# evenrose/CMDIAD

Measured on AMD Instinct MI355X. Metric: images/sec end-to-end (extract+distill+kNN score), higher is better.
Workload: dtype bf16; 1 GPU; configs[1]: DINO ViT-B/8 + Point-MAE predict (DoubleRGBPointFeatures: both modalities are extracted, this method has no distillation step at test time; the `mtfi_step` leg times the method that has one), 224x224 RGB + 24576-point clouds (1024 groups x 128), batch 32/GPU, bagel-sized banks (xyz 76518x768, rgb 19129x768); batch_per_gpu=32, rotating_input_batches=4, bank=single, hip_graphs=True, search_operands=bf16 (fp32 accumulate, exact fp32 re-score of the winner), weights=seeded random init (no checkpoints offline)

## Files before the change

cmdiad_amd/csrc/mlp_fused.hip:

```cpp
#include "gemm_core.h"
#include "launch.h"

namespace {

using namespace gemm;

constexpr int kC = 384, kHid = 1536, kBM = 128, kWaves = 8;
constexpr int kChunks = kHid / 64;
constexpr int kKT1 = kC / BK;
constexpr int kPer = kKT1 + kC / 64;
constexpr int kSlots = 6, kAhead = kSlots - 1;
static_assert(kPer % kSlots == 0, "the slot of a piece depends on its place in the chunk only");
constexpr int kPieceBytes = 64 * BK * 2;
constexpr int kXbWave = kKT1 * 16 * BK * 2;
constexpr int kHOff = kWaves * kXbWave;
constexpr int kRingOff = kHOff + kWaves * 2048;
constexpr int kLdsBytes = kRingOff + kSlots * kPieceBytes;
static_assert(kLdsBytes == 160 * 1024, "LDS budget");

struct MlpParams {
    int M;
    const bf16_t* xb;
    const float* row_scale;
    const bf16_t* w1;
    const float* b1;
    const bf16_t* w2;
    const float* b2;
    float* x;
    bf16_t* ln_xb;
    float* ln_part;
    const float* add2;
};

__device__ __forceinline__ void mlp_barrier() { asm volatile("s_barrier" ::: "memory"); }

__device__ __forceinline__ float half_row_sum8(float v)
{
    v += __builtin_bit_cast(float, __builtin_amdgcn_update_dpp(0, __builtin_bit_cast(int, v), 0xB1, 0xF, 0xF, false));
    v += __builtin_bit_cast(float, __builtin_amdgcn_update_dpp(0, __builtin_bit_cast(int, v), 0x4E, 0xF, 0xF, false));
    v += __builtin_bit_cast(float, __builtin_amdgcn_update_dpp(0, __builtin_bit_cast(int, v), 0x141, 0xF, 0xF, false));
    return v;
}

template <bool LN_OUT>
__global__ __launch_bounds__(512, 1) void pmae_mlp_fused_kernel(MlpParams p)
{
    extern __shared__ __attribute__((aligned(16))) char lds[];
    const int lane = threadIdx.x & 63, wave = __builtin_amdgcn_readfirstlane(threadIdx.x >> 6);
    const int g = lane >> 4, r16 = lane & 15;
    const int mw = (int)blockIdx.x * kBM + wave * 16;
    char* xs = lds + wave * kXbWave;
    char* hs = lds + kHOff + wave * 2048;
    char* ring = lds + kRingOff;

    float rsc;
    f32x4 b1v[4];
    auto load_b1 = [&](int c) {
        const float* bp = p.b1 + c * 64 + g * 4;
#pragma unroll
        for (int j = 0; j < 4; ++j) asm volatile("global_load_dwordx4 %0, %1, off" : "=v"(b1v[j]) : "v"(bp + j * 16) : "memory");
    };
    {
        const float* rp = p.row_scale + min(mw + r16, p.M - 1);
        asm volatile("global_load_dword %0, %1, off" : "=v"(rsc) : "v"(rp) : "memory");
    }
    load_b1(0);
    const int sw_chunk = (lane & 7) ^ (lane >> 3);
#pragma unroll
    for (int e = 0; e < 2; ++e) {
        const bf16_t* src = p.xb + (size_t)min(mw + e * 8 + (lane >> 3), p.M - 1) * kC + sw_chunk * 8;
#pragma unroll
        for (int s = 0; s < kKT1; ++s)
            __builtin_amdgcn_global_load_lds((const __attribute__((address_space(1))) void*)(src + s * BK),
                                             (__attribute__((address_space(3))) void*)(xs + s * 2048 + e * 1024), 16, 0, 0);
    }
    const char* w1l = reinterpret_cast<const char*>(p.w1 + (size_t)(wave * 8 + (lane >> 3)) * kC + sw_chunk * 8);
    const char* w2l = reinterpret_cast<const char*>(p.w2 + (size_t)(wave * 8 + (lane >> 3)) * kHid + sw_chunk * 8);
    auto issue = [&](int c, int q) {
        const char* src = q < kKT1 ? w1l + ((size_t)c * 64 * kC + q * BK) * 2 : w2l + ((size_t)(q - kKT1) * 64 * kHid + c * BK) * 2;
        __builtin_amdgcn_global_load_lds((const __attribute__((address_space(1))) void*)src,
                                         (__attribute__((address_space(3))) void*)(ring + (q % kSlots) * kPieceBytes + wave * 1024), 16, 0, 0);
    };
#pragma unroll
    for (int q = 0; q < kAhead; ++q) issue(0, q);
    asm volatile("s_waitcnt vmcnt(4)" ::: "memory");
    mlp_barrier();

    auto ldf = [&](const char* tile, int row, int kk) { return *reinterpret_cast<const bf16x8*>(tile + lds_off(row, kk * 4 + g)); };
    auto step = [&](const char* wt, const bf16x8& a0, const bf16x8& a1, f32x4 (&acc)[4]) {
        bf16x8 wf[2][4];
#pragma unroll
        for (int kk = 0; kk < 2; ++kk)
#pragma unroll
            for (int j = 0; j < 4; ++j) wf[kk][j] = ldf(wt, j * 16 + r16, kk);
        __builtin_amdgcn_s_setprio(1);
#pragma unroll
        for (int kk = 0; kk < 2; ++kk)
#pragma unroll
            for (int j = 0; j < 4; ++j) acc[j] = mfma16(wf[kk][j], kk ? a1 : a0, acc[j]);
        __builtin_amdgcn_s_setprio(0);
    };

    f32x4 acc2[kC / 64][4];
#pragma unroll
    for (int nb = 0; nb < kC / 64; ++nb)
#pragma unroll
        for (int j = 0; j < 4; ++j) acc2[nb][j] = f32x4{0.f, 0.f, 0.f, 0.f};

    for (int c = 0; c < kChunks; ++c) {
        f32x4 acc1[4];
#pragma unroll
        for (int j = 0; j < 4; ++j) acc1[j] = f32x4{0.f, 0.f, 0.f, 0.f};
        bf16x8 h0, h1;
#pragma unroll
        for (int q = 0; q < kPer; ++q) {
            const int qn = q + kAhead < kPer ? q + kAhead : q + kAhead - kPer;
            const int cn = q + kAhead < kPer ? c : c + 1;
            const bool more = cn < kChunks;
            if (q == 7 && more) load_b1(c + 1);
            if (more) issue(cn, qn);
            const char* wt = ring + (q % kSlots) * kPieceBytes;
            if (q < kKT1) step(wt, ldf(xs + q * 2048, r16, 0), ldf(xs + q * 2048, r16, 1), acc1);
            else step(wt, h0, h1, acc2[q - kKT1]);
            if (!more) asm volatile("s_waitcnt vmcnt(0)" ::: "memory");
            else if (q >= 7 && q <= 10) asm volatile("s_waitcnt vmcnt(8)" ::: "memory");
            else asm volatile("s_waitcnt vmcnt(4)" ::: "memory");
            mlp_barrier();
            if (q == kKT1 - 1) {
                __builtin_amdgcn_sched_barrier(0);
#pragma unroll
                for (int j = 0; j < 4; ++j) {
                    f32x4 v = __builtin_elementwise_fma(acc1[j], f32x4{rsc, rsc, rsc, rsc}, b1v[j]);
                    v = gelu_erf4(v);
                    const bf16x4 hv = {f2bf(v[0]), f2bf(v[1]), f2bf(v[2]), f2bf(v[3])};
                    *reinterpret_cast<bf16x4*>(hs + lds_off(r16, 2 * j + (g >> 1)) + (g & 1) * 8) = hv;
                }
                h0 = ldf(hs, r16, 0);
                h1 = ldf(hs, r16, 1);
            }
        }
    }

    RowStore32 rs;
    rs.init(hs, lane);
    const bool full = mw + 16 <= p.M;
    const int m0r = mw + rs.R;
    const int ma = min(m0r, p.M - 1), mb = min(m0r + 8, p.M - 1);
#pragma unroll
    for (int nb = 0; nb < kC / 64; ++nb) {
        const int n0 = nb * 64;
        f32x4 bj[4];
#pragma unroll
        for (int j = 0; j < 4; ++j) bj[j] = *reinterpret_cast<const f32x4*>(p.b2 + n0 + j * 16 + g * 4);
        f32x4 o0[2], o1[2];
#pragma unroll
        for (int ch = 0; ch < 2; ++ch) {
            const int col = n0 + ch * 32 + rs.u * 4;
            const f32x4 r0 = *reinterpret_cast<const f32x4*>(p.x + (size_t)ma * kC + col);
            const f32x4 r1 = *reinterpret_cast<const f32x4*>(p.x + (size_t)mb * kC + col);
            f32x4 a0 = {0.f, 0.f, 0.f, 0.f}, a1 = a0;
            if (LN_OUT && p.add2) {
                a0 = *reinterpret_cast<const f32x4*>(p.add2 + (size_t)ma * kC + col);
                a1 = *reinterpret_cast<const f32x4*>(p.add2 + (size_t)mb * kC + col);
            }
            rs.park(acc2[nb][2 * ch] + bj[2 * ch], acc2[nb][2 * ch + 1] + bj[2 * ch + 1]);
            f32x4 t0, t1;
            rs.fetch(t0, t1);
            o0[ch] = t0 + r0;
            o1[ch] = t1 + r1;
            if (LN_OUT && p.add2) { o0[ch] += a0; o1[ch] += a1; }
            if (full || m0r < p.M) *reinterpret_cast<f32x4*>(p.x + (size_t)m0r * kC + col) = o0[ch];
            if (full || m0r + 8 < p.M) *reinterpret_cast<f32x4*>(p.x + (size_t)(m0r + 8) * kC + col) = o1[ch];
            if constexpr (LN_OUT) {
                const bf16x4 v0 = {f2bf(o0[ch][0]), f2bf(o0[ch][1]), f2bf(o0[ch][2]), f2bf(o0[ch][3])};
                const bf16x4 v1 = {f2bf(o1[ch][0]), f2bf(o1[ch][1]), f2bf(o1[ch][2]), f2bf(o1[ch][3])};
                if (full || m0r < p.M) *reinterpret_cast<bf16x4*>(p.ln_xb + (size_t)m0r * kC + col) = v0;
                if (full || m0r + 8 < p.M) *reinterpret_cast<bf16x4*>(p.ln_xb + (size_t)(m0r + 8) * kC + col) = v1;
            }
        }
        if constexpr (LN_OUT) {
            float s0 = 0.f, s1 = 0.f;
#pragma unroll
            for (int ch = 0; ch < 2; ++ch)
#pragma unroll
                for (int q = 0; q < 4; ++q) { s0 += o0[ch][q]; s1 += o1[ch][q]; }
            s0 = half_row_sum8(s0);
            s1 = half_row_sum8(s1);
            const float c0 = s0 * (1.0f / 64), c1 = s1 * (1.0f / 64);
            float q0 = 0.f, q1 = 0.f;
#pragma unroll
            for (int ch = 0; ch < 2; ++ch)
#pragma unroll
                for (int q = 0; q < 4; ++q) {
                    const float d0 = o0[ch][q] - c0, d1 = o1[ch][q] - c1;
                    q0 = fmaf(d0, d0, q0);
                    q1 = fmaf(d1, d1, q1);
                }
            q0 = half_row_sum8(q0);
            q1 = half_row_sum8(q1);
            if (rs.u == 0) {
                float2* part = reinterpret_cast<float2*>(p.ln_part) + (size_t)nb * p.M;
                if (full || m0r < p.M) part[m0r] = make_float2(s0, q0);
                if (full || m0r + 8 < p.M) part[m0r + 8] = make_float2(s1, q1);
            }
        }
    }
}

}

int cmdiad_pmae_mlp_fused(float* x, const uint16_t* xb, const float* rstd, const uint16_t* w1, const float* b1, const uint16_t* w2,
                          const float* b2, int M, uint16_t* ln_xb, float* ln_part, const float* add2, cmdiad_stream_t stream)
{
    CMDIAD_REQUIRE(x && xb && rstd && w1 && b1 && w2 && b2 && M > 0, CMDIAD_ERR_ARG, "cmdiad_pmae_mlp_fused: null operand");
    CMDIAD_REQUIRE(aligned16(x) && aligned16(xb) && aligned16(w1) && aligned16(w2) && aligned16(b1) && aligned16(b2) && (!add2 || aligned16(add2)), CMDIAD_ERR_ARG,
                   "cmdiad_pmae_mlp_fused: operands must be 16-byte aligned");
    CMDIAD_REQUIRE(!ln_xb == !ln_part && (ln_xb || !add2) && (!ln_xb || (((uintptr_t)ln_xb & 7) == 0 && ((uintptr_t)ln_part & 7) == 0)),
                   CMDIAD_ERR_ARG, "cmdiad_pmae_mlp_fused: ln_xb and ln_part come together (8-byte aligned); add2 only with them");
    MlpParams p{M, (const bf16_t*)xb, rstd, (const bf16_t*)w1, b1, (const bf16_t*)w2, b2, x, (bf16_t*)ln_xb, ln_part, add2};
    const dim3 grid((unsigned)((M + kBM - 1) / kBM)), block(kWaves * 64);
    const int rc = ln_xb ? launch_lds<pmae_mlp_fused_kernel<true>>("cmdiad_pmae_mlp_fused", grid, block, kLdsBytes, (hipStream_t)stream, p)
                         : launch_lds<pmae_mlp_fused_kernel<false>>("cmdiad_pmae_mlp_fused", grid, block, kLdsBytes, (hipStream_t)stream, p);
    if (rc) return rc;
    CMDIAD_CHECK_LAUNCH();
    return CMDIAD_OK;
}
```

Baseline: 1601 images/s.

## Halve waves in fused Point-MAE MLP, two row blocks per wave with fragment prefetch

The fused MLP kernel now runs 4 waves instead of 8, and each wave owns 32 rows (two 16-row blocks). Every weight fragment read from LDS therefore feeds twice as many MFMAs. Weight and activation fragments for the next piece are read from LDS into a ping-pong register set before the current piece's MFMAs run, and the ring prefetch depth and counted waits are adjusted to match. The aim is to cut LDS read traffic per MFMA and hide LDS latency. The cost is higher register pressure from doubled accumulators, and fewer waves left to hide memory latency.

```diff
diff --git a/cmdiad_amd/csrc/mlp_fused.hip b/cmdiad_amd/csrc/mlp_fused.hip
--- a/cmdiad_amd/csrc/mlp_fused.hip
+++ b/cmdiad_amd/csrc/mlp_fused.hip
@@ -5,16 +5,21 @@
 
 using namespace gemm;
 
-constexpr int kC = 384, kHid = 1536, kBM = 128, kWaves = 8;
+constexpr int kC = 384, kHid = 1536, kBM = 128, kWaves = 4;
+constexpr int kRB = kBM / kWaves / 16;
 constexpr int kChunks = kHid / 64;
 constexpr int kKT1 = kC / BK;
 constexpr int kPer = kKT1 + kC / 64;
-constexpr int kSlots = 6, kAhead = kSlots - 1;
+constexpr int kSlots = 6;
 static_assert(kPer % kSlots == 0, "the slot of a piece depends on its place in the chunk only");
+static_assert(kPer % 2 == 0, "the fragment ping-pong is indexed by a piece's place in the chunk");
 constexpr int kPieceBytes = 64 * BK * 2;
-constexpr int kXbWave = kKT1 * 16 * BK * 2;
+constexpr int kGl = 64 / kWaves / 8;
+static_assert(kGl == 2, "the counted waits below are written for two instructions per piece");
+constexpr int kXbTile = kRB * 16 * BK * 2;
+constexpr int kXbWave = kKT1 * kXbTile;
 constexpr int kHOff = kWaves * kXbWave;
-constexpr int kRingOff = kHOff + kWaves * 2048;
+constexpr int kRingOff = kHOff + kWaves * kRB * 2048;
 constexpr int kLdsBytes = kRingOff + kSlots * kPieceBytes;
 static_assert(kLdsBytes == 160 * 1024, "LDS budget");
 
@@ -32,7 +37,11 @@
     const float* add2;
 };
 
-__device__ __forceinline__ void mlp_barrier() { asm volatile("s_barrier" ::: "memory"); }
+__device__ __forceinline__ void mlp_barrier()
+{
+    __builtin_amdgcn_s_waitcnt(0xC07F);
+    asm volatile("s_barrier" ::: "memory");
+}
 
 __device__ __forceinline__ float half_row_sum8(float v)
 {
@@ -43,165 +52,202 @@
 }
 
 template <bool LN_OUT>
-__global__ __launch_bounds__(512, 1) void pmae_mlp_fused_kernel(MlpParams p)
+__global__ __launch_bounds__(256, 1) void pmae_mlp_fused_kernel(MlpParams p)
 {
     extern __shared__ __attribute__((aligned(16))) char lds[];
     const int lane = threadIdx.x & 63, wave = __builtin_amdgcn_readfirstlane(threadIdx.x >> 6);
     const int g = lane >> 4, r16 = lane & 15;
-    const int mw = (int)blockIdx.x * kBM + wave * 16;
+    const int mw = (int)blockIdx.x * kBM + wave * (kRB * 16);
     char* xs = lds + wave * kXbWave;
-    char* hs = lds + kHOff + wave * 2048;
+    char* hs = lds + kHOff + wave * (kRB * 2048);
     char* ring = lds + kRingOff;
 
-    float rsc;
+    float rsc[kRB];
     f32x4 b1v[4];
     auto load_b1 = [&](int c) {
         const float* bp = p.b1 + c * 64 + g * 4;
 #pragma unroll
         for (int j = 0; j < 4; ++j) asm volatile("global_load_dwordx4 %0, %1, off" : "=v"(b1v[j]) : "v"(bp + j * 16) : "memory");
     };
-    {
-        const float* rp = p.row_scale + min(mw + r16, p.M - 1);
-        asm volatile("global_load_dword %0, %1, off" : "=v"(rsc) : "v"(rp) : "memory");
+#pragma unroll
+    for (int b = 0; b < kRB; ++b) {
+        const float* rp = p.row_scale + min(mw + b * 16 + r16, p.M - 1);
+        asm volatile("global_load_dword %0, %1, off" : "=v"(rsc[b]) : "v"(rp) : "memory");
     }
     load_b1(0);
     const int sw_chunk = (lane & 7) ^ (lane >> 3);
 #pragma unroll
-    for (int e = 0; e < 2; ++e) {
+    for (int e = 0; e < kRB * 2; ++e) {
         const bf16_t* src = p.xb + (size_t)min(mw + e * 8 + (lane >> 3), p.M - 1) * kC + sw_chunk * 8;
 #pragma unroll
         for (int s = 0; s < kKT1; ++s)
             __builtin_amdgcn_global_load_lds((const __attribute__((address_space(1))) void*)(src + s * BK),
-                                             (__attribute__((address_space(3))) void*)(xs + s * 2048 + e * 1024), 16, 0, 0);
-    }
-    const char* w1l = reinterpret_cast<const char*>(p.w1 + (size_t)(wave * 8 + (lane >> 3)) * kC + sw_chunk * 8);
-    const char* w2l = reinterpret_cast<const char*>(p.w2 + (size_t)(wave * 8 + (lane >> 3)) * kHid + sw_chunk * 8);
+                                             (__attribute__((address_space(3))) void*)(xs + s * kXbTile + e * 1024), 16, 0, 0);
+    }
+    const char* w1l = reinterpret_cast<const char*>(p.w1 + (size_t)(wave * 16 + (lane >> 3)) * kC + sw_chunk * 8);
+    const char* w2l = reinterpret_cast<const char*>(p.w2 + (size_t)(wave * 16 + (lane >> 3)) * kHid + sw_chunk * 8);
     auto issue = [&](int c, int q) {
         const char* src = q < kKT1 ? w1l + ((size_t)c * 64 * kC + q * BK) * 2 : w2l + ((size_t)(q - kKT1) * 64 * kHid + c * BK) * 2;
-        __builtin_amdgcn_global_load_lds((const __attribute__((address_space(1))) void*)src,
-                                         (__attribute__((address_space(3))) void*)(ring + (q % kSlots) * kPieceBytes + wave * 1024), 16, 0, 0);
-    };
-#pragma unroll
-    for (int q = 0; q < kAhead; ++q) issue(0, q);
-    asm volatile("s_waitcnt vmcnt(4)" ::: "memory");
+        const size_t ld = (q < kKT1 ? kC : kHid) * 2;
+#pragma unroll
+        for (int e = 0; e < kGl; ++e)
+            __builtin_amdgcn_global_load_lds((const __attribute__((address_space(1))) void*)(src + e * 8 * ld),
+                                             (__attribute__((address_space(3))) void*)(ring + (q % kSlots) * kPieceBytes + (wave * kGl + e) * 1024),
+                                             16, 0, 0);
+    };
+#pragma unroll
+    for (int q = 0; q < kSlots; ++q) issue(0, q);
+    asm volatile("s_waitcnt vmcnt(8)" ::: "memory");
     mlp_barrier();
 
     auto ldf = [&](const char* tile, int row, int kk) { return *reinterpret_cast<const bf16x8*>(tile + lds_off(row, kk * 4 + g)); };
-    auto step = [&](const char* wt, const bf16x8& a0, const bf16x8& a1, f32x4 (&acc)[4]) {
-        bf16x8 wf[2][4];
+    bf16x8 wf[2][2][4];
+    bf16x8 xf[2][kRB][2];
+    auto read_w = [&](int q, bf16x8 (&w)[2][4]) {
+        const char* wt = ring + (q % kSlots) * kPieceBytes;
 #pragma unroll
         for (int kk = 0; kk < 2; ++kk)
 #pragma unroll
-            for (int j = 0; j < 4; ++j) wf[kk][j] = ldf(wt, j * 16 + r16, kk);
-        __builtin_amdgcn_s_setprio(1);
-#pragma unroll
-        for (int kk = 0; kk < 2; ++kk)
-#pragma unroll
-            for (int j = 0; j < 4; ++j) acc[j] = mfma16(wf[kk][j], kk ? a1 : a0, acc[j]);
-        __builtin_amdgcn_s_setprio(0);
-    };
-
-    f32x4 acc2[kC / 64][4];
-#pragma unroll
-    for (int nb = 0; nb < kC / 64; ++nb)
-#pragma unroll
-        for (int j = 0; j < 4; ++j) acc2[nb][j] = f32x4{0.f, 0.f, 0.f, 0.f};
+            for (int j = 0; j < 4; ++j) w[kk][j] = ldf(wt, j * 16 + r16, kk);
+    };
+    auto read_x = [&](int s, bf16x8 (&x)[kRB][2]) {
+#pragma unroll
+        for (int b = 0; b < kRB; ++b)
+#pragma unroll
+            for (int kk = 0; kk < 2; ++kk) x[b][kk] = ldf(xs + s * kXbTile, b * 16 + r16, kk);
+    };
+    read_w(0, wf[0]);
+    read_x(0, xf[0]);
+    mlp_barrier();
+
+    f32x4 acc2[kRB][kC / 64][4];
+#pragma unroll
+    for (int b = 0; b < kRB; ++b)
+#pragma unroll
+        for (int nb = 0; nb < kC / 64; ++nb)
+#pragma unroll
+            for (int j = 0; j < 4; ++j) acc2[b][nb][j] = f32x4{0.f, 0.f, 0.f, 0.f};
 
     for (int c = 0; c < kChunks; ++c) {
-        f32x4 acc1[4];
-#pragma unroll
-        for (int j = 0; j < 4; ++j) acc1[j] = f32x4{0.f, 0.f, 0.f, 0.f};
-        bf16x8 h0, h1;
+        f32x4 acc1[kRB][4];
+#pragma unroll
+        for (int b = 0; b < kRB; ++b)
+#pragma unroll
+            for (int j = 0; j < 4; ++j) acc1[b][j] = f32x4{0.f, 0.f, 0.f, 0.f};
+        bf16x8 hf[kRB][2];
 #pragma unroll
         for (int q = 0; q < kPer; ++q) {
-            const int qn = q + kAhead < kPer ? q + kAhead : q + kAhead - kPer;
-            const int cn = q + kAhead < kPer ? c : c + 1;
+            const int qn = q + kSlots < kPer ? q + kSlots : q + kSlots - kPer;
+            const int cn = q + kSlots < kPer ? c : c + 1;
             const bool more = cn < kChunks;
             if (q == 7 && more) load_b1(c + 1);
             if (more) issue(cn, qn);
-            const char* wt = ring + (q % kSlots) * kPieceBytes;
-            if (q < kKT1) step(wt, ldf(xs + q * 2048, r16, 0), ldf(xs + q * 2048, r16, 1), acc1);
-            else step(wt, h0, h1, acc2[q - kKT1]);
+            const int q1 = q + 1 < kPer ? q + 1 : 0;
+            if (q + 1 < kPer || c + 1 < kChunks) {
+                read_w(q1, wf[q1 & 1]);
+                if (q1 < kKT1) read_x(q1, xf[q1 & 1]);
+            }
+            __builtin_amdgcn_sched_barrier(0);
+            __builtin_amdgcn_s_setprio(1);
+#pragma unroll
+            for (int kk = 0; kk < 2; ++kk)
+#pragma unroll
+                for (int b = 0; b < kRB; ++b)
+#pragma unroll
+                    for (int j = 0; j < 4; ++j) {
+                        if (q < kKT1) acc1[b][j] = mfma16(wf[q & 1][kk][j], xf[q & 1][b][kk], acc1[b][j]);
+                        else acc2[b][q - kKT1][j] = mfma16(wf[q & 1][kk][j], hf[b][kk], acc2[b][q - kKT1][j]);
+                    }
+            __builtin_amdgcn_s_setprio(0);
+            __builtin_amdgcn_sched_barrier(0);
             if (!more) asm volatile("s_waitcnt vmcnt(0)" ::: "memory");
-            else if (q >= 7 && q <= 10) asm volatile("s_waitcnt vmcnt(8)" ::: "memory");
-            else asm volatile("s_waitcnt vmcnt(4)" ::: "memory");
+            else if (q >= 7 && q <= 10) asm volatile("s_waitcnt vmcnt(12)" ::: "memory");
+            else asm volatile("s_waitcnt vmcnt(8)" ::: "memory");
             mlp_barrier();
             if (q == kKT1 - 1) {
                 __builtin_amdgcn_sched_barrier(0);
 #pragma unroll
-                for (int j = 0; j < 4; ++j) {
-                    f32x4 v = __builtin_elementwise_fma(acc1[j], f32x4{rsc, rsc, rsc, rsc}, b1v[j]);
-                    v = gelu_erf4(v);
-                    const bf16x4 hv = {f2bf(v[0]), f2bf(v[1]), f2bf(v[2]), f2bf(v[3])};
-                    *reinterpret_cast<bf16x4*>(hs + lds_off(r16, 2 * j + (g >> 1)) + (g & 1) * 8) = hv;
-                }
-                h0 = ldf(hs, r16, 0);
-                h1 = ldf(hs, r16, 1);
+                for (int b = 0; b < kRB; ++b) {
+                    char* hb = hs + b * 2048;
+#pragma unroll
+                    for (int j = 0; j < 4; ++j) {
+                        f32x4 v = __builtin_elementwise_fma(acc1[b][j], f32x4{rsc[b], rsc[b], rsc[b], rsc[b]}, b1v[j]);
+                        v = gelu_erf4(v);
+                        const bf16x4 hv = {f2bf(v[0]), f2bf(v[1]), f2bf(v[2]), f2bf(v[3])};
+                        *reinterpret_cast<bf16x4*>(hb + lds_off(r16, 2 * j + (g >> 1)) + (g & 1) * 8) = hv;
+                    }
+                    hf[b][0] = ldf(hb, r16, 0);
+                    hf[b][1] = ldf(hb, r16, 1);
+                }
             }
         }
     }
 
     RowStore32 rs;
     rs.init(hs, lane);
-    const bool full = mw + 16 <= p.M;
-    const int m0r = mw + rs.R;
-    const int ma = min(m0r, p.M - 1), mb = min(m0r + 8, p.M - 1);
-#pragma unroll
-    for (int nb = 0; nb < kC / 64; ++nb) {
-        const int n0 = nb * 64;
-        f32x4 bj[4];
-#pragma unroll
-        for (int j = 0; j < 4; ++j) bj[j] = *reinterpret_cast<const f32x4*>(p.b2 + n0 + j * 16 + g * 4);
-        f32x4 o0[2], o1[2];
-#pragma unroll
-        for (int ch = 0; ch < 2; ++ch) {
-            const int col = n0 + ch * 32 + rs.u * 4;
-            const f32x4 r0 = *reinterpret_cast<const f32x4*>(p.x + (size_t)ma * kC + col);
-            const f32x4 r1 = *reinterpret_cast<const f32x4*>(p.x + (size_t)mb * kC + col);
-            f32x4 a0 = {0.f, 0.f, 0.f, 0.f}, a1 = a0;
-            if (LN_OUT && p.add2) {
-                a0 = *reinterpret_cast<const f32x4*>(p.add2 + (size_t)ma * kC + col);
-                a1 = *reinterpret_cast<const f32x4*>(p.add2 + (size_t)mb * kC + col);
-            }
-            rs.park(acc2[nb][2 * ch] + bj[2 * ch], acc2[nb][2 * ch + 1] + bj[2 * ch + 1]);
-            f32x4 t0, t1;
-            rs.fetch(t0, t1);
-            o0[ch] = t0 + r0;
-            o1[ch] = t1 + r1;
-            if (LN_OUT && p.add2) { o0[ch] += a0; o1[ch] += a1; }
-            if (full || m0r < p.M) *reinterpret_cast<f32x4*>(p.x + (size_t)m0r * kC + col) = o0[ch];
-            if (full || m0r + 8 < p.M) *reinterpret_cast<f32x4*>(p.x + (size_t)(m0r + 8) * kC + col) = o1[ch];
+#pragma unroll
+    for (int b = 0; b < kRB; ++b) {
+        const int mb0 = mw + b * 16;
+        const bool full = mb0 + 16 <= p.M;
+        const int m0r = mb0 + rs.R;
+        const int ma = min(m0r, p.M - 1), mb = min(m0r + 8, p.M - 1);
+#pragma unroll
+        for (int nb = 0; nb < kC / 64; ++nb) {
+            const int n0 = nb * 64;
+            f32x4 bj[4];
+#pragma unroll
+            for (int j = 0; j < 4; ++j) bj[j] = *reinterpret_cast<const f32x4*>(p.b2 + n0 + j * 16 + g * 4);
+            f32x4 o0[2], o1[2];
+#pragma unroll
+            for (int ch = 0; ch < 2; ++ch) {
+                const int col = n0 + ch * 32 + rs.u * 4;
+                const f32x4 r0 = *reinterpret_cast<const f32x4*>(p.x + (size_t)ma * kC + col);
+                const f32x4 r1 = *reinterpret_cast<const f32x4*>(p.x + (size_t)mb * kC + col);
+                f32x4 a0 = {0.f, 0.f, 0.f, 0.f}, a1 = a0;
+                if (LN_OUT && p.add2) {
+                    a0 = *reinterpret_cast<const f32x4*>(p.add2 + (size_t)ma * kC + col);
+                    a1 = *reinterpret_cast<const f32x4*>(p.add2 + (size_t)mb * kC + col);
+                }
+                rs.park(acc2[b][nb][2 * ch] + bj[2 * ch], acc2[b][nb][2 * ch + 1] + bj[2 * ch + 1]);
+                f32x4 t0, t1;
+                rs.fetch(t0, t1);
+                o0[ch] = t0 + r0;
+                o1[ch] = t1 + r1;
+                if (LN_OUT && p.add2) { o0[ch] += a0; o1[ch] += a1; }
+                if (full || m0r < p.M) *reinterpret_cast<f32x4*>(p.x + (size_t)m0r * kC + col) = o0[ch];
+                if (full || m0r + 8 < p.M) *reinterpret_cast<f32x4*>(p.x + (size_t)(m0r + 8) * kC + col) = o1[ch];
+                if constexpr (LN_OUT) {
+                    const bf16x4 v0 = {f2bf(o0[ch][0]), f2bf(o0[ch][1]), f2bf(o0[ch][2]), f2bf(o0[ch][3])};
+                    const bf16x4 v1 = {f2bf(o1[ch][0]), f2bf(o1[ch][1]), f2bf(o1[ch][2]), f2bf(o1[ch][3])};
+                    if (full || m0r < p.M) *reinterpret_cast<bf16x4*>(p.ln_xb + (size_t)m0r * kC + col) = v0;
+                    if (full || m0r + 8 < p.M) *reinterpret_cast<bf16x4*>(p.ln_xb + (size_t)(m0r + 8) * kC + col) = v1;
+                }
+            }
             if constexpr (LN_OUT) {
-                const bf16x4 v0 = {f2bf(o0[ch][0]), f2bf(o0[ch][1]), f2bf(o0[ch][2]), f2bf(o0[ch][3])};
-                const bf16x4 v1 = {f2bf(o1[ch][0]), f2bf(o1[ch][1]), f2bf(o1[ch][2]), f2bf(o1[ch][3])};
-                if (full || m0r < p.M) *reinterpret_cast<bf16x4*>(p.ln_xb + (size_t)m0r * kC + col) = v0;
-                if (full || m0r + 8 < p.M) *reinterpret_cast<bf16x4*>(p.ln_xb + (size_t)(m0r + 8) * kC + col) = v1;
-            }
-        }
-        if constexpr (LN_OUT) {
-            float s0 = 0.f, s1 = 0.f;
-#pragma unroll
-            for (int ch = 0; ch < 2; ++ch)
-#pragma unroll
-                for (int q = 0; q < 4; ++q) { s0 += o0[ch][q]; s1 += o1[ch][q]; }
-            s0 = half_row_sum8(s0);
-            s1 = half_row_sum8(s1);
-            const float c0 = s0 * (1.0f / 64), c1 = s1 * (1.0f / 64);
-            float q0 = 0.f, q1 = 0.f;
-#pragma unroll
-            for (int ch = 0; ch < 2; ++ch)
-#pragma unroll
-                for (int q = 0; q < 4; ++q) {
-                    const float d0 = o0[ch][q] - c0, d1 = o1[ch][q] - c1;
-                    q0 = fmaf(d0, d0, q0);
-                    q1 = fmaf(d1, d1, q1);
-                }
-            q0 = half_row_sum8(q0);
-            q1 = half_row_sum8(q1);
-            if (rs.u == 0) {
-                float2* part = reinterpret_cast<float2*>(p.ln_part) + (size_t)nb * p.M;
-                if (full || m0r < p.M) part[m0r] = make_float2(s0, q0);
-                if (full || m0r + 8 < p.M) part[m0r + 8] = make_float2(s1, q1);
+                float s0 = 0.f, s1 = 0.f;
+#pragma unroll
+                for (int ch = 0; ch < 2; ++ch)
+#pragma unroll
+                    for (int q = 0; q < 4; ++q) { s0 += o0[ch][q]; s1 += o1[ch][q]; }
+                s0 = half_row_sum8(s0);
+                s1 = half_row_sum8(s1);
+                const float c0 = s0 * (1.0f / 64), c1 = s1 * (1.0f / 64);
+                float q0 = 0.f, q1 = 0.f;
+#pragma unroll
+                for (int ch = 0; ch < 2; ++ch)
+#pragma unroll
+                    for (int q = 0; q < 4; ++q) {
+                        const float d0 = o0[ch][q] - c0, d1 = o1[ch][q] - c1;
+                        q0 = fmaf(d0, d0, q0);
+                        q1 = fmaf(d1, d1, q1);
+                    }
+                q0 = half_row_sum8(q0);
+                q1 = half_row_sum8(q1);
+                if (rs.u == 0) {
+                    float2* part = reinterpret_cast<float2*>(p.ln_part) + (size_t)nb * p.M;
+                    if (full || m0r < p.M) part[m0r] = make_float2(s0, q0);
+                    if (full || m0r + 8 < p.M) part[m0r + 8] = make_float2(s1, q1);
+                }
             }
         }
     }
```

Result: no change. 1598 images/s (-0.2%).
